# gabry1998/Self-Supervised-Anomaly-Detection

Measured on AMD Instinct MI355X. Metric: train images/sec + anomaly-maps/sec, ResNet-18 256x256 bs256, higher is better.
Workload: dtype f32; 1 GPU; ResNet-18 256x256 bs256 self-sup train + anomaly map, 1xMI355X, synthetic images (BASELINE configs[1]); images_per_gpu=256, global_batch=256, patches_per_image=841, bank_rows=588, parallelism=dp1 (256 images), train_step_launch=hipGraph segments, train_graph_segments=1

## Files before the change

include/ssad.h:

```cpp
#ifndef SSAD_H
#define SSAD_H
#include <stddef.h>
#include <stdint.h>

#ifdef __cplusplus
extern "C" {
#endif

#define SSAD_VERSION 100

int ssad_version(void);
const char* ssad_last_error(void);

int ssad_repack_oihw_to_ohwi(const float* w_oihw, float* w_ohwi, int O, int I, int KH, int KW, void* stream);
int ssad_repack_ohwi_to_oihw(const float* w_ohwi, float* w_oihw, int O, int I, int KH, int KW, void* stream);
int ssad_pack_stem_weight(const float* w_oihw, float* wk, void* stream);
int ssad_pack_stem_weight_ohwi(const float* w_ohwi, float* wk, void* stream);

int ssad_stem_fwd(const float* img, int B, int H, int W, int patch_dim, int patch_stride, int Hv, int Wv,
                  const float* wk, const float* scale, const float* shift, int relu, int hwnc, float* out, void* stream);
int ssad_stem_stats_rows(void);
int ssad_stem_fwd_stats(const float* img, int B, int H, int W, int Hv, int Wv, const float* wk, float* out, float eps,
                        float momentum, float* mean, float* invstd, float* running_mean, float* running_var, double* workspace,
                        void* stream);
// ... 3 lines not shown
                             const float* shift, int hwnc, float* out, void* stream);
int ssad_stem_patch_pool_fwd_ring(const float* img, int B, int H, int W, int patch_stride, const float* wf, const float* scale,
                                  const float* shift, int hwnc, int skip_lo, int skip_hi, float* out, void* stream);
int ssad_stem_patch_border_fwd(const float* img, int B, int H, int W, int patch_stride, const float* wf, const float* scale,
                               const float* shift, float* out, void* stream);

int ssad_maxpool3x3s2_fwd(const float* in, float* out, int64_t N, int H, int W, int C, int hwnc, void* stream);

int ssad_conv_igemm_fwd(const float* in, const float* w_ohwi, float* out, const float* scale, const float* shift,
                        const float* residual, int relu, int64_t N, int H, int W, int Cin, int Cout, int KH, int KW,
                        int stride, int pad, void* stream);

int ssad_conv_igemm_fwd_hwnc(const float* in, const float* w_ohwi, float* out, const float* scale, const float* shift,
                             const float* residual, int relu, int64_t N, int H, int W, int Cin, int Cout, int KH, int KW,
                             int stride, int pad, void* stream);

int ssad_conv_igemm_fwd_hwnc_ring(const float* in, const float* w_ohwi, float* out, const float* scale, const float* shift,
                                  const float* residual, int relu, int64_t N, int H, int W, int Cin, int Cout, int KH, int KW,
                                  int stride, int pad, int skip_lo, int skip_hi, void* stream);
int ssad_patch_gather_hwnc(const float* dense, float* out, int64_t B, int prow, int pcol, int shift, int Hd, int Wd, int C,
                           int H, int W, int lo, int hi, void* stream);
int ssad_patch_gather_hwnc_band(const float* dense, float* out, int64_t B, int prow, int pcol, int shift, int Hd, int Wd, int C,
                                int H, int W, int lo, int hi, int ilo, int ihi, void* stream);

int ssad_conv_igemm_tile(int64_t N, int H, int W, int Cin, int Cout, int KH, int KW, int stride, int pad, int mode);
int ssad_conv_igemm_tile_id(int64_t N, int H, int W, int Cin, int Cout, int KH, int KW, int stride, int pad, int mode);

int ssad_gap_fwd(const float* in, float* out, int64_t N, int HW, int C, int out_stride, int out_offset, int hwnc,
                 void* stream);

int ssad_l2_normalize_rows(const float* x, float* out, int64_t N, int D, void* stream);
int ssad_cosine_knn_mean(const float* sim, float* out, int64_t Nq, int Nb, int k, void* stream);

int ssad_blur_relu_bilinear(const float* maps, float* out, int n, int h, int w, int ksize, int target, void* stream);

int ssad_gradcam_map(const float* act, const float* alpha, float* out, int64_t B, int HW, int C, int alpha_stride,
                     void* stream);

int64_t ssad_auroc_workspace(int64_t n);
int ssad_auroc(const float* scores, const uint8_t* labels, int64_t n, void* workspace, int64_t workspace_bytes, double* out,
               void* stream);

int ssad_flip_transpose_weight(const float* w_ohwi, float* out, int O, int I, int KH, int KW, void* stream);
int ssad_flip_transpose_batch(const float* src, float* dst, const int64_t* desc, int n, void* stream);
int ssad_conv_igemm_dgrad(const float* dy, const float* w_flipT, float* dx, const float* residual, int64_t N, int Hy, int Wy,
                          int Cout, int Hx, int Wx, int Cin, int KH, int KW, int stride, int pad, void* stream);
// ... 310 lines not shown
```

self-supervised-anomaly-detection_amd/csrc/conv_igemm.hip:

```cpp
#include "common.h"
#include <stdlib.h>
#include <type_traits>

#ifndef IGEMM_ABL
#define IGEMM_ABL 0
#endif
#ifndef IGEMM_VAR
#define IGEMM_VAR 4
#endif
#ifndef IGEMM_EPI
#define IGEMM_EPI 1
#endif


#ifndef IGEMM_BUFLD
#define IGEMM_BUFLD 1
#endif

#ifndef IGEMM_TRACE
#define IGEMM_TRACE 0
#endif
#if IGEMM_TRACE
__device__ unsigned long long* g_ig_trace;
#define IG_STAMP(i) do { if (threadIdx.x == 0 && g_ig_trace) g_ig_trace[((size_t)blockIdx.y * gridDim.x + blockIdx.x) * 8 + (i)] = __builtin_readcyclecounter(); } while (0)
// ... 4 lines not shown
namespace {

constexpr int KALIGN = 32;

__device__ __attribute__((aligned(16))) float g_zero_page[8] = {0, 0, 0, 0, 0, 0, 0, 0};

struct ConvParams {
    const float* in;
    const float* wt;
    float* out;
    const float* scale;
    const float* shift;
    const float* residual;
    const uint8_t* res_mask;
    int64_t M;
    int64_t N;
    int H, W, Cin, Ho, Wo, Cout, KH, KW, stride, pad, relu;
    int K;
    int hwnc;
    int cls_start[5];
    int cls_id[4];
    double* stats;
    int skip_lo, skip_hi;
    int pos_lpt;
    int pos_sg;
    int pos_chunk;
    unsigned char pos_tab[64];
};

template <int BM, int BN, int TM, int TN, int BK, int TS, bool POS, bool DB = true, int BF = 0, bool IO = false>
__global__ __launch_bounds__((BM / (32 * TM)) * (BN / (32 * TN)) * 64, (TM * TN > 8 || (TM * TN == 8 && BK >= 32)) ? 1 : 2)
void conv_igemm_f32_kernel(ConvParams p) {
    static_assert(!IO || BF == 2, "half tensors go with fp16 operands");
    using io_t = std::conditional_t<IO, hf, float>;
    constexpr int PE = IO ? 8 : 4;
    constexpr int NT = (BM / (32 * TM)) * (BN / (32 * TN)) * 64;
    constexpr int LDK = BF == 6 ? 3 * BK + 8 : (BF == 3 ? 2 * BK + 8 : (BF ? BK + 8 : BK + 4));
    constexpr int ESZ = BF ? 2 : 4;
    constexpr int CPR = BK / PE;
    constexpr int RPP = NT / CPR;
    constexpr int WN = BN / (32 * TN);
    constexpr int AR = BM / RPP;
    constexpr int BR = BN / RPP;
    static_assert(AR >= 1 && BR >= 1, "tile too small for the staging pattern");
    constexpr int STAGE = (BM + BN) * LDK * ESZ / 4;
    constexpr int LDC = BN + 4;
// ... 29 lines not shown
            const unsigned pi = r / (unsigned)p.pos_chunk, g = r - pi * (unsigned)p.pos_chunk;
            const unsigned sg = (blk * (unsigned)p.pos_chunk + g) * 8u + x;
            if (sg >= (unsigned)p.pos_sg) return;
            pos = p.pos_tab[pi];
            m0 = (int64_t)sg * BM;
        } else if (p.pos_lpt) {
            const unsigned per_chunk = (unsigned)p.pos_chunk * (unsigned)HoWo;
            const unsigned chunk = blockIdx.x / per_chunk, in_chunk = blockIdx.x - chunk * per_chunk;
            const unsigned first = chunk * (unsigned)p.pos_chunk;
            const unsigned here = min((unsigned)p.pos_chunk, (unsigned)p.pos_sg - first);
            const unsigned pi = in_chunk / here;
            if (pi >= (unsigned)HoWo) return;
            pos = p.pos_tab[pi];
            m0 = (int64_t)(first + in_chunk - pi * here) * BM;
        } else {
        const int stream = blockIdx.x & 31;
        const int64_t j = blockIdx.x >> 5;
        const int64_t q = j / HoWo;
        pos = (int)(j - q * HoWo);
        m0 = (q * 32 + stream) * BM;
        }
        if (m0 >= p.N) return;
        const int oy = pos / p.Wo, ox = pos - oy * p.Wo;
        if (oy >= p.skip_lo && oy <= p.skip_hi && ox >= p.skip_lo && ox <= p.skip_hi) return;
        tapmask = 0;
        for (int ky = 0, t = 0; ky < p.KH; ++ky)
            for (int kx = 0; kx < p.KW; ++kx, ++t) {
                const int y = oy * p.stride - p.pad + ky, x = ox * p.stride - p.pad + kx;
                if ((unsigned)y < (unsigned)p.H && (unsigned)x < (unsigned)p.W) tapmask |= 1u << t;
            }
    } else {
        m0 = (int64_t)blockIdx.x * BM;
    }
    int cpy = 0, cpx = 0, Hc = 1, Wc = 1;
    int64_t Mc = 0;
    if (TS > 1) {
        int c = 0;
        while (c < 3 && (int)blockIdx.x >= p.cls_start[c + 1]) ++c;
        cpy = p.cls_id[c] >> 1;
        cpx = p.cls_id[c] & 1;
        Hc = (p.Ho - cpy + 1) / 2;
        Wc = (p.Wo - cpx + 1) / 2;
        Mc = p.N * Hc * Wc;
        m0 = (int64_t)((int)blockIdx.x - p.cls_start[c]) * BM;
        tapmask = 0;
        for (int ky = 0, t = 0; ky < p.KH; ++ky)
            for (int kx = 0; kx < p.KW; ++kx, ++t)
// ... 803 lines not shown
        return launch<128, 128, 2, 2, 32, TS, POS, false, 6>(p, st);
    }
    if (p.Cout <= 64) return launch<256, 64, 2, 2, 16, TS, POS, true, 6>(p, st);
    return launch<128, 128, 2, 2, 16, TS, POS, true, 6>(p, st);
}

template <int TS, bool POS>
int dispatch_x3(const ConvParams& p, hipStream_t st) {
    static const int v = getenv("SSAD_X3_VARIANT") ? atoi(getenv("SSAD_X3_VARIANT")) : 1;
    if (v == 1) {
        if (p.Cout <= 64) return launch<256, 64, 2, 2, 32, TS, POS, false, 3>(p, st);
        return launch<128, 128, 2, 2, 32, TS, POS, false, 3>(p, st);
    }
    if (p.Cout <= 64) return launch<256, 64, 2, 2, 16, TS, POS, true, 3>(p, st);
    return launch<128, 128, 2, 2, 32, TS, POS, true, 3>(p, st);
}

enum IgemmTile { T_256x64_K16 = 0, T_256x64_SB, T_128x64, T_256x128, T_256x128_W4, T_128x256, T_64x64, T_128x128, T_256x256, T_128x64_SB, T_128x64_K16, T_128x128_K16, T_128x256_K16 };

template <bool POS>
IgemmTile pick_tile(const ConvParams& p) {
    static const int variant = getenv("SSAD_CONV64_VARIANT") ? atoi(getenv("SSAD_CONV64_VARIANT")) : 1;
    static const int ring = getenv("SSAD_CONV_RING_VARIANT") ? atoi(getenv("SSAD_CONV_RING_VARIANT")) : 0;
    if (p.Cout <= 64 && POS && p.skip_lo <= p.skip_hi && !getenv("SSAD_CONV64_VARIANT"))
        return ring == 1 ? T_128x64_SB : ring == 3 ? T_128x64 : T_128x64_K16;
    if (p.Cout <= 64) return variant == 2 ? T_256x64_SB : variant == 1 ? T_256x64_K16 : T_128x64;
    static const int big = getenv("SSAD_CONV128_VARIANT") ? atoi(getenv("SSAD_CONV128_VARIANT")) : 0;
    if (big == 7) return T_128x128_K16;
    if (big == 1) return T_256x128;
    if (big == 2) return T_256x128_W4;
    if (big == 6 && POS && p.Cout % 256 == 0 && cdiv64(p.N, 256) * p.Ho * p.Wo * (p.Cout / 256) >= 256) return T_256x256;
    static const int wide_min = getenv("SSAD_CONV_WIDE_GRID") ? atoi(getenv("SSAD_CONV_WIDE_GRID")) : 256;
    if (big != 5 && p.Cout % 256 == 0 && wide_min > 0) {
        const int64_t rows = POS ? cdiv64(p.N, 128) * p.Ho * p.Wo : cdiv64(p.M, 128);
        static const int wide_k16 = getenv("SSAD_CONV256_K16") ? atoi(getenv("SSAD_CONV256_K16")) : 2;
        if (rows * (p.Cout / 256) >= wide_min) return (wide_k16 == 2 || (POS && wide_k16)) ? T_128x256_K16 : T_128x256;
    }
    static const int small_min = getenv("SSAD_CONV_SMALL_GRID") ? atoi(getenv("SSAD_CONV_SMALL_GRID")) : 500;
    static const int tiny_min = getenv("SSAD_CONV_TINY_GRID") ? atoi(getenv("SSAD_CONV_TINY_GRID")) : 520;
    if (!POS) {
        const int64_t g128 = cdiv64(p.M, 128) * ((p.Cout + 127) / 128);
        if (cdiv64(p.M, 128) * ((p.Cout + 63) / 64) < tiny_min && p.M > 128) return T_64x64;
        if (g128 < small_min) return T_128x64;
    }
    static const int k16 = getenv("SSAD_CONV128_K16") ? atoi(getenv("SSAD_CONV128_K16")) : 1;
    if (POS && k16) return T_128x128_K16;
    return T_128x128;
// ... 10 lines not shown
        case T_128x128_K16: return launch<128, 128, 2, 2, 16, TS, POS>(p, st);
        case T_128x256_K16: return launch<128, 256, 2, 4, 16, TS, POS>(p, st);
        case T_256x128: return launch<256, 128, 2, 2, 32, TS, POS>(p, st);
        case T_256x128_W4: return launch<256, 128, 4, 2, 32, TS, POS>(p, st);
        case T_128x256: return launch<128, 256, 2, 4, 32, TS, POS>(p, st);
        case T_64x64: return launch<64, 64, 1, 1, 32, TS, POS>(p, st);
        case T_256x256:
            if constexpr (POS && TS == 1) return launch<256, 256, 4, 4, 32, TS, POS>(p, st);
            else return launch<128, 128, 2, 2, 32, TS, POS>(p, st);
        default: return launch<128, 128, 2, 2, 32, TS, POS>(p, st);
    }
}

enum IgemmEntry { E_FWD = 0, E_HWNC = 1, E_RING = 2, E_STATS = 3, E_DGRAD = 4 };

static bool posmajor_rows(IgemmEntry e, const ConvParams& p) {
    if (e == E_HWNC || e == E_RING) return true;
    return e == E_FWD && p.pad > 0 && p.N >= 128 && p.Ho * p.Wo <= 4;
}

static ConvParams dgrad_params(int64_t N, int Hy, int Wy, int Cout, int Hx, int Wx, int Cin, int KH, int KW, int pad) {
    ConvParams p;
    p.pos_lpt = 0; p.pos_sg = 0; p.pos_chunk = 1;
    p.skip_lo = 1; p.skip_hi = 0;
    p.in = nullptr; p.wt = nullptr; p.out = nullptr; p.scale = nullptr; p.shift = nullptr; p.residual = nullptr; p.res_mask = nullptr;
    p.H = Hy; p.W = Wy; p.Cin = Cout; p.Cout = Cin; p.KH = KH; p.KW = KW; p.relu = 0;
    p.stride = 1; p.pad = KH - 1 - pad; p.N = N; p.hwnc = 0;
    p.Ho = Hx; p.Wo = Wx; p.stats = nullptr;
    p.M = N * Hx * Wx;
    p.K = KH * KW * Cout;
    return p;
}

static bool tile_span_ok(const ConvParams& p, bool posmajor, int elt_bytes, int ts = 1) {
    const int64_t image = (int64_t)p.H * p.W * p.Cin * elt_bytes;
    if (posmajor) return p.hwnc || 256 * image < ((int64_t)1 << 31);
    const int64_t rows_per_image = ts > 1 ? (int64_t)(p.Ho / 2) * (p.Wo / 2) : (int64_t)p.Ho * p.Wo;
    return (256 / (rows_per_image > 0 ? rows_per_image : 1) + 2) * image < ((int64_t)1 << 31);
}

int conv_fwd_impl(const float* in, const float* w_ohwi, float* out, const float* scale, const float* shift,
                  const float* residual, int relu, int64_t N, int H, int W, int Cin, int Cout, int KH, int KW, int stride,
                  int pad, int hwnc, void* stream, int bf16 = 0, double* stats = nullptr, int* stat_rows = nullptr, int io16 = 0,
                  int skip_lo = 1, int skip_hi = 0) {
    SSAD_CHECK_ARG(in && w_ohwi && out, "null pointer");
    SSAD_CHECK_ARG(!io16 || (bf16 == 2 && !hwnc && Cout % 4 == 0), "half tensors: fp16 operands, NHWC, Cout % 4 == 0");
    SSAD_CHECK_ARG(N > 0 && H > 0 && W > 0 && Cin > 0 && Cout > 0, "empty shape");
    if ((bf16 == 0 || bf16 == 1 || bf16 == 2) && !io16 && !hwnc && KH == 1 && KW == 1 && H == 1 && W == 1 && stride == 1 && pad == 0 &&
        ssad_linear_small_ok(in, w_ohwi, N, Cin))
        return ssad_linear_small_launch(in, w_ohwi, out, scale, shift, residual, relu, (int)N, Cin, Cout, stats, stat_rows, stream, bf16);
    SSAD_CHECK_ARG(Cin % KALIGN == 0, "Cin must be a multiple of 32");
    SSAD_CHECK_ARG(KH > 0 && KW > 0 && stride > 0 && pad >= 0 && KH * KW <= 32, "bad filter geometry (<= 32 taps)");
    ConvParams p;
    p.pos_lpt = 0; p.pos_sg = 0; p.pos_chunk = 1;
    p.skip_lo = skip_lo; p.skip_hi = skip_hi;
    SSAD_CHECK_ARG(skip_lo > skip_hi || hwnc, "a skipped rectangle of output positions: position-major tensors only");
    p.in = in; p.wt = w_ohwi; p.out = out; p.scale = scale; p.shift = shift; p.residual = residual; p.res_mask = nullptr;
    p.H = H; p.W = W; p.Cin = Cin; p.Cout = Cout; p.KH = KH; p.KW = KW; p.stride = stride; p.pad = pad; p.relu = relu;
    p.Ho = (H + 2 * pad - KH) / stride + 1;
    p.Wo = (W + 2 * pad - KW) / stride + 1;
    SSAD_CHECK_ARG(p.Ho > 0 && p.Wo > 0, "empty output");
    p.M = N * p.Ho * p.Wo;
    p.N = N;
    p.K = KH * KW * Cin;
    p.hwnc = hwnc;
    p.stats = stats;
    const bool posmajor = posmajor_rows(hwnc ? (skip_lo <= skip_hi ? E_RING : E_HWNC) : stats ? E_STATS : E_FWD, p);
    SSAD_CHECK_ARG(cdiv64(p.M, 128) + 32 * p.Ho * p.Wo < (int64_t)2147483647, "M too large for one launch");
    SSAD_CHECK_ARG(tile_span_ok(p, posmajor, io16 ? 2 : 4), "input images too large: the rows of a tile must span less than 2 GB");
    hipStream_t st = (hipStream_t)stream;
    int rows;
    SSAD_CHECK_ARG(bf16 == 0 || bf16 == 1 || bf16 == 2 || bf16 == 3 || bf16 == 6,
                   "operand mode: 0 (fp32), 1 (bf16), 2 (fp16), 3 (bf16x3), 6 (bf16x6)");
    if (bf16 == 6) {
        rows = posmajor ? dispatch_x6<1, true>(p, st) : dispatch_x6<1, false>(p, st);
    } else if (bf16 == 3) {
        rows = posmajor ? dispatch_x3<1, true>(p, st) : dispatch_x3<1, false>(p, st);
    } else if (bf16) {
        SSAD_CHECK_ARG(!hwnc, "16-bit operands: NHWC only");
        rows = io16 ? dispatch_bf16<1, 2, true>(p, st) : bf16 == 2 ? dispatch_bf16<1, 2>(p, st) : dispatch_bf16<1, 1>(p, st);
    } else if (posmajor) rows = dispatch<1, true>(p, st);
    else rows = dispatch<1, false>(p, st);
    if (stat_rows) *stat_rows = rows;
    SSAD_CHECK_LAUNCH();
    return 0;
}

}

extern "C" int ssad_conv_igemm_fwd_bf16(const float* in, const float* w_ohwi, float* out, const float* scale,
// ... 39 lines not shown
    int rc = conv_fwd_impl(in, w_ohwi, out, nullptr, nullptr, nullptr, 0, N, H, W, Cin, Cout, KH, KW, stride, pad, 0, stream,
                           bf16, workspace, &rows);
    if (rc) return rc;
    const int Ho = (H + 2 * pad - KH) / stride + 1, Wo = (W + 2 * pad - KW) / stride + 1;
    return ssad_bn_finalize_partials(workspace, rows, N * Ho * Wo, Cout, eps, momentum, mean, invstd, running_mean,
                                     running_var, stream);
}

extern "C" int ssad_conv_igemm_fwd_hwnc(const float* in, const float* w_ohwi, float* out, const float* scale,
                                        const float* shift, const float* residual, int relu, int64_t N, int H, int W,
                                        int Cin, int Cout, int KH, int KW, int stride, int pad, void* stream) {
    return conv_fwd_impl(in, w_ohwi, out, scale, shift, residual, relu, N, H, W, Cin, Cout, KH, KW, stride, pad, 1, stream);
}

extern "C" int ssad_conv_igemm_fwd_hwnc_ring(const float* in, const float* w_ohwi, float* out, const float* scale,
                                             const float* shift, const float* residual, int relu, int64_t N, int H, int W,
                                             int Cin, int Cout, int KH, int KW, int stride, int pad, int skip_lo, int skip_hi,
                                             void* stream) {
    SSAD_CHECK_ARG(skip_lo >= 0 && skip_hi < H && skip_hi < W, "skipped square outside the map");
    return conv_fwd_impl(in, w_ohwi, out, scale, shift, residual, relu, N, H, W, Cin, Cout, KH, KW, stride, pad, 1, stream, 0, nullptr,
                         nullptr, 0, skip_lo, skip_hi);
}

extern "C" int ssad_conv_igemm_tile_id(int64_t N, int H, int W, int Cin, int Cout, int KH, int KW, int stride, int pad, int mode) {
    const int Ho = (H + 2 * pad - KH) / stride + 1, Wo = (W + 2 * pad - KW) / stride + 1;
    ConvParams p;
    if (mode == E_DGRAD) {
        p = dgrad_params(N, Ho, Wo, Cout, H, W, Cin, KH, KW, pad);
    } else {
        p.N = N; p.H = H; p.W = W; p.Cin = Cin; p.Cout = Cout; p.KH = KH; p.KW = KW; p.stride = stride; p.pad = pad;
        p.skip_lo = mode == E_RING ? 0 : 1; p.skip_hi = 0;
        p.Ho = Ho; p.Wo = Wo;
        p.M = N * p.Ho * p.Wo;
    }
    if (posmajor_rows((IgemmEntry)mode, p)) return 100 + (int)pick_tile<true>(p);
    const IgemmTile t = pick_tile<false>(p);
    return t == T_256x256 ? T_128x128 : (int)t;
}

extern "C" int ssad_conv_igemm_tile(int64_t N, int H, int W, int Cin, int Cout, int KH, int KW, int stride, int pad, int mode) {
    static const int dims[13][3] = {{256, 64, 16}, {256, 64, 32}, {128, 64, 32}, {256, 128, 32}, {256, 128, 32}, {128, 256, 32},
                                    {64, 64, 32}, {128, 128, 32}, {256, 256, 32}, {128, 64, 32}, {128, 64, 16}, {128, 128, 16}, {128, 256, 16}};
    const int id = ssad_conv_igemm_tile_id(N, H, W, Cin, Cout, KH, KW, stride, pad, mode), t = id % 100;
    const int code = dims[t][0] * 100000 + dims[t][1] * 100 + dims[t][2];
    return id >= 100 ? -code : code;
}

static int dgrad_impl(const float* dy, const float* w_flipT, float* dx, const float* residual, int64_t N,
                                     int Hy, int Wy, int Cout, int Hx, int Wx, int Cin, int KH, int KW, int stride,
                                     int pad, void* stream, int bf16, const uint8_t* res_mask = nullptr, int io16 = 0) {
    SSAD_CHECK_ARG(dy && w_flipT && dx, "null pointer");
    SSAD_CHECK_ARG(!io16 || (bf16 == 2 && !res_mask && Cin % 4 == 0), "half tensors: fp16 operands, no residual mask, Cin % 4 == 0");
    SSAD_CHECK_ARG(N > 0 && Hy > 0 && Wy > 0 && Hx > 0 && Wx > 0 && Cin > 0 && Cout > 0, "empty shape");
    if ((bf16 == 0 || bf16 == 1 || bf16 == 2) && !io16 && !res_mask && KH == 1 && KW == 1 && Hy == 1 && Wy == 1 && Hx == 1 && Wx == 1 &&
// ... 95 lines not shown
```

self-supervised-anomaly-detection_amd/csrc/misc.hip:

```cpp
#include "common.h"
#include <stdarg.h>

static thread_local char g_err[512] = "";

void ssad_set_error(const char* fmt, ...) {
    va_list ap;
    va_start(ap, fmt);
    vsnprintf(g_err, sizeof(g_err), fmt, ap);
    va_end(ap);
}

extern "C" const char* ssad_last_error(void) { return g_err; }
extern "C" int ssad_version(void) { return 100; }

namespace {

__global__ void repack_kernel(const float* __restrict__ src, float* __restrict__ dst, int O, int I, int KH, int KW,
                              int to_ohwi) {
    int64_t idx = (int64_t)blockIdx.x * blockDim.x + threadIdx.x;
    int64_t total = (int64_t)O * I * KH * KW;
    if (idx >= total) return;
    int ci = (int)(idx % I);
    int64_t t = idx / I;
    int kx = (int)(t % KW); t /= KW;
// ... 297 lines not shown
}

extern "C" int ssad_patch_gather_hwnc_band(const float* dense, float* out, int64_t B, int prow, int pcol, int shift, int Hd, int Wd, int C,
                                           int H, int W, int lo, int hi, int ilo, int ihi, void* stream) {
    SSAD_CHECK_ARG(dense && out && B > 0 && prow > 0 && pcol > 0 && shift > 0 && C > 0 && C % 4 == 0, "bad argument");
    SSAD_CHECK_ARG(lo >= 0 && hi >= lo && hi < H && hi < W, "the copied square must lie inside the map");
    SSAD_CHECK_ARG(ilo > ihi || (ilo > lo && ihi < hi), "the inner square must lie strictly inside the copied one");
    SSAD_CHECK_ARG(shift * (prow - 1) + hi < Hd && shift * (pcol - 1) + hi < Wd, "the dense map does not cover the last patch");
    const int64_t N = B * prow * pcol;
    const int side = hi - lo + 1;
    const int iside = ilo > ihi ? 0 : ihi - ilo + 1;
    SSAD_CHECK_ARG(cdiv64(N * (C / 4), 256) < (int64_t)2147483647 && side * side <= 65535, "too large for one launch");
    hipLaunchKernelGGL(patch_gather_hwnc_kernel, dim3((unsigned)cdiv64(N * (C / 4), 256), side * side - iside * iside), dim3(256), 0,
                       (hipStream_t)stream, (const f32x4*)dense, (f32x4*)out, N, prow, pcol, shift, Hd, Wd, C / 4, W, lo, side, ilo, iside);
    SSAD_CHECK_LAUNCH();
    return 0;
}

extern "C" int ssad_patch_gather_hwnc(const float* dense, float* out, int64_t B, int prow, int pcol, int shift, int Hd, int Wd, int C,
                                      int H, int W, int lo, int hi, void* stream) {
    return ssad_patch_gather_hwnc_band(dense, out, B, prow, pcol, shift, Hd, Wd, C, H, W, lo, hi, 1, 0, stream);
}

extern "C" int ssad_gradcam_map(const float* act, const float* alpha, float* out, int64_t B, int HW, int C, int alpha_stride,
                                void* stream) {
    SSAD_CHECK_ARG(act && alpha && out && B > 0 && HW > 0 && C > 0 && alpha_stride >= C, "bad argument");
    const int64_t rows = B * HW;
    hipLaunchKernelGGL(gradcam_map_kernel, dim3((unsigned)cdiv64(rows, 4)), dim3(256), 0, (hipStream_t)stream, act, alpha, out,
                       rows, HW, C, alpha_stride);
    SSAD_CHECK_LAUNCH();
    return 0;
}

extern "C" int ssad_l2_normalize_rows(const float* x, float* out, int64_t N, int D, void* stream) {
    SSAD_CHECK_ARG(x && out && N > 0 && D > 0, "bad argument");
    hipLaunchKernelGGL(l2norm_rows_kernel, dim3((unsigned)cdiv64(N, 4)), dim3(256), 0, (hipStream_t)stream, x, out, N, D);
    SSAD_CHECK_LAUNCH();
    return 0;
}

extern "C" int ssad_cosine_knn_mean(const float* sim, float* out, int64_t Nq, int Nb, int k, void* stream) {
    SSAD_CHECK_ARG(sim && out && Nq > 0 && Nb > 0, "bad argument");
    SSAD_CHECK_ARG(k >= 1 && k <= 3 && k <= Nb, "k must be 1..3 and <= bank rows");
    hipLaunchKernelGGL(knn_mean_kernel, dim3((unsigned)cdiv64(Nq, 4)), dim3(256), 0, (hipStream_t)stream, sim, out, Nq, Nb, k);
    SSAD_CHECK_LAUNCH();
    return 0;
// ... 25 lines not shown
```

self-supervised-anomaly-detection_amd/self_supervised/_hip.py:

```python
import ctypes
import os

import torch

_HERE = os.path.dirname(os.path.abspath(__file__))
LIB_PATH = os.path.join(os.path.dirname(_HERE), "lib", "libssad_hip.so")

_c_fp = ctypes.c_void_p
_c_i = ctypes.c_int
_c_l = ctypes.c_int64
_c_f = ctypes.c_float

SIGNATURES = {
    "ssad_repack_oihw_to_ohwi": [_c_fp, _c_fp, _c_i, _c_i, _c_i, _c_i, _c_fp],
    "ssad_repack_ohwi_to_oihw": [_c_fp, _c_fp, _c_i, _c_i, _c_i, _c_i, _c_fp],
    "ssad_pack_stem_weight": [_c_fp, _c_fp, _c_fp],
    "ssad_pack_stem_weight_ohwi": [_c_fp, _c_fp, _c_fp],
    "ssad_pack_stem_weight16_ohwi": [_c_fp, _c_fp, _c_i, _c_fp],
    "ssad_stem_fwd": [_c_fp, _c_i, _c_i, _c_i, _c_i, _c_i, _c_i, _c_i, _c_fp, _c_fp, _c_fp, _c_i, _c_i, _c_fp, _c_fp],
    "ssad_stem_stats_rows": [],
    "ssad_stem_fwd_stats": [_c_fp, _c_i, _c_i, _c_i, _c_i, _c_i, _c_fp, _c_fp, _c_f, _c_f, _c_fp, _c_fp, _c_fp, _c_fp, _c_fp, _c_fp],
    "ssad_pack_stem_weight_folded": [_c_fp, _c_fp, _c_fp],
    "ssad_stem_patch_pool_fwd": [_c_fp, _c_i, _c_i, _c_i, _c_i, _c_fp, _c_fp, _c_fp, _c_i, _c_fp, _c_fp],
    "ssad_stem_patch_pool_fwd_ring": [_c_fp, _c_i, _c_i, _c_i, _c_i, _c_fp, _c_fp, _c_fp, _c_i, _c_i, _c_i, _c_fp, _c_fp],
    "ssad_stem_patch_border_fwd": [_c_fp, _c_i, _c_i, _c_i, _c_i, _c_fp, _c_fp, _c_fp, _c_fp, _c_fp],
    "ssad_maxpool3x3s2_fwd": [_c_fp, _c_fp, _c_l, _c_i, _c_i, _c_i, _c_i, _c_fp],
    "ssad_conv_igemm_fwd": [_c_fp, _c_fp, _c_fp, _c_fp, _c_fp, _c_fp, _c_i, _c_l, _c_i, _c_i, _c_i, _c_i, _c_i, _c_i,
                            _c_i, _c_i, _c_fp],
    "ssad_conv_igemm_fwd_hwnc": [_c_fp, _c_fp, _c_fp, _c_fp, _c_fp, _c_fp, _c_i, _c_l, _c_i, _c_i, _c_i, _c_i, _c_i, _c_i,
                                 _c_i, _c_i, _c_fp],
    "ssad_conv_igemm_fwd_hwnc_ring": [_c_fp, _c_fp, _c_fp, _c_fp, _c_fp, _c_fp, _c_i, _c_l, _c_i, _c_i, _c_i, _c_i, _c_i, _c_i,
                                      _c_i, _c_i, _c_i, _c_i, _c_fp],
    "ssad_patch_gather_hwnc": [_c_fp, _c_fp, _c_l, _c_i, _c_i, _c_i, _c_i, _c_i, _c_i, _c_i, _c_i, _c_i, _c_i, _c_fp],
    "ssad_patch_gather_hwnc_band": [_c_fp, _c_fp, _c_l, _c_i, _c_i, _c_i, _c_i, _c_i, _c_i, _c_i, _c_i, _c_i, _c_i, _c_i, _c_i, _c_fp],
    "ssad_conv_igemm_tile": [_c_l, _c_i, _c_i, _c_i, _c_i, _c_i, _c_i, _c_i, _c_i, _c_i],
    "ssad_conv_igemm_tile_id": [_c_l, _c_i, _c_i, _c_i, _c_i, _c_i, _c_i, _c_i, _c_i, _c_i],
    "ssad_gap_fwd": [_c_fp, _c_fp, _c_l, _c_i, _c_i, _c_i, _c_i, _c_i, _c_fp],
    "ssad_l2_normalize_rows": [_c_fp, _c_fp, _c_l, _c_i, _c_fp],
    "ssad_cosine_knn_mean": [_c_fp, _c_fp, _c_l, _c_i, _c_i, _c_fp],
    "ssad_cosine_knn_fused": [_c_fp, _c_fp, _c_fp, _c_l, _c_i, _c_i, _c_i, _c_fp],
    "ssad_cosine_knn_split": [_c_fp, _c_fp, _c_fp, _c_fp, _c_l, _c_i, _c_i, _c_i, _c_i, _c_fp],
    "ssad_cosine_knn_index": [_c_fp, _c_fp, _c_fp, _c_fp, _c_l, _c_i, _c_i, _c_i, _c_fp],
    "ssad_cosine_knn_index_split": [_c_fp, _c_fp, _c_fp, _c_fp, _c_fp, _c_l, _c_i, _c_i, _c_i, _c_i, _c_fp],
    "ssad_rows_smallest_index": [_c_fp, _c_l, _c_i, _c_i, _c_i, _c_i, _c_fp, _c_fp, _c_fp, _c_fp],
    "ssad_rows_argmax": [_c_fp, _c_l, _c_i, _c_fp, _c_fp, _c_fp],
    "ssad_knn_reweight": [_c_fp, _c_fp, _c_fp, _c_fp, _c_fp, _c_fp, _c_l, _c_i, _c_i, _c_i, _c_fp],
    "ssad_row_sqnorms": [_c_fp, _c_fp, _c_l, _c_i, _c_fp],
    "ssad_l2_knn_fused": [_c_fp, _c_fp, _c_fp, _c_fp, _c_l, _c_i, _c_i, _c_i, _c_fp],
    "ssad_l2_knn_split": [_c_fp, _c_fp, _c_fp, _c_fp, _c_fp, _c_l, _c_i, _c_i, _c_i, _c_i, _c_fp],
    "ssad_l2_knn_index": [_c_fp, _c_fp, _c_fp, _c_fp, _c_fp, _c_l, _c_i, _c_i, _c_i, _c_fp],
    "ssad_l2_knn_index_split": [_c_fp, _c_fp, _c_fp, _c_fp, _c_fp, _c_fp, _c_l, _c_i, _c_i, _c_i, _c_i, _c_fp],
    "ssad_l2_from_dots": [_c_fp, _c_fp, _c_fp, _c_fp, _c_l, _c_i, _c_fp],
    "ssad_knn_reweight_l2": [_c_fp, _c_fp, _c_fp, _c_fp, _c_fp, _c_fp, _c_l, _c_i, _c_i, _c_i, _c_fp],
    "ssad_local_patch_features": [_c_fp, _c_fp, _c_fp, _c_l, _c_i, _c_i, _c_i, _c_i, _c_i, _c_i, _c_i, _c_fp],
    "ssad_coreset_greedy": [_c_fp, _c_l, _c_i, _c_i, _c_l, _c_i, _c_fp, _c_fp, _c_fp, _c_fp, _c_fp, _c_fp],
# ... 215 lines not shown
```

self-supervised-anomaly-detection_amd/self_supervised/engine.py:

```python
import torch
from torch import nn

import os as _os

from . import ops

BLOCKS = [("layer1", 64, 64, 1), ("layer2", 64, 128, 2), ("layer3", 128, 256, 2), ("layer4", 256, 512, 2)]


def math_mode():
    m = _os.environ.get("SSAD_MATH", "f32").lower()
    return 6 if m in ("bf16x6", "x6") else 3 if m in ("bf16x3", "x3") else 0


class _Block(nn.Module):

    def __init__(self, cin, cout, stride):
        super().__init__()
        self.conv1 = nn.Conv2d(cin, cout, 3, stride, 1, bias=False)
        self.bn1 = nn.BatchNorm2d(cout)
        self.conv2 = nn.Conv2d(cout, cout, 3, 1, 1, bias=False)
        self.bn2 = nn.BatchNorm2d(cout)
        self.downsample = None
        if stride != 1 or cin != cout:
# ... 126 lines not shown
        if last_of_stage and maps is not None and name in maps:
            maps[name] = a
    return pooled


def _trunk_eval_dedup(plan, x, patch_stride, layer_outputs, pooled, conv):
    b, _, h, w = x.shape
    prow, pcol = (h - 32) // patch_stride + 1, (w - 32) // patch_stride + 1
    shift = patch_stride // 2
    band = _os.environ.get("SSAD_GATHER_BAND", "1") != "0"
    dn = ops.stem_fwd(x, plan.stem_w, plan.stem_s, plan.stem_t, True, resize_to=(2 * h, 2 * w))
    dn = ops.maxpool3x3s2_fwd(dn)
    if band and _os.environ.get("SSAD_STEM_BORDER", "1") != "0":
        a = ops.stem_patch_border_fwd(x, plan.stem_wf, plan.stem_s, plan.stem_t, patch_stride)
        ops.patch_gather_hwnc(dn, a, prow, pcol, shift, 2, 14, 4, 12)
    else:
        a = ops.stem_patch_pool_fwd(x, plan.stem_wf, plan.stem_s, plan.stem_t, patch_stride, True, (4, 12) if band else None)
    offs, off = {}, 0
    for k in ("layer1", "layer2", "layer3"):
        if k in layer_outputs:
            offs[k] = off
            off += {"layer1": 64, "layer2": 128, "layer3": 256}[k]
    offs["layer4"] = off
    for i, (name, d) in enumerate(plan.blocks):
        s = d["stride"]
        if name == "layer1":
            lo, hi = 3 + 2 * i, 13 - 2 * i
            dt = ops.conv3x3_c64_eval(dn, d["w1"], d["s1"], d["t1"], None, True)
            dn2 = ops.conv3x3_c64_eval(dt, d["w2"], d["s2"], d["t2"], dn, True)
            t = ops.conv_fwd_hwnc_ring(a, d["w1"], d["s1"], d["t1"], None, True, lo, hi)
            ops.patch_gather_hwnc(dt, t, prow, pcol, shift, lo, hi, *((lo + 2, hi - 2) if band else (1, 0)))
            a2 = ops.conv_fwd_hwnc_ring(t, d["w2"], d["s2"], d["t2"], a, True, lo + 1, hi - 1)
            ops.patch_gather_hwnc(dn2, a2, prow, pcol, shift, lo + 1, hi - 1, *((lo + 3, hi - 3) if band and i == 0 else (1, 0)))
            a, dn = a2, dn2
        else:
            idt = a
            if "wd" in d:
                idt = conv(a, d["wd"], d["sd"], d["td"], None, False, s, 0)
            t = conv(a, d["w1"], d["s1"], d["t1"], None, True, s, 1)
            a = conv(t, d["w2"], d["s2"], d["t2"], idt, True, 1, 1)
        if i % 2 == 1 and name in offs:
            ops.gap_fwd(a, pooled, offs[name], True)
    return pooled


def head_eval(plan, pooled):
    f = pooled
    x3 = math_mode()
    for w, s, t, relu in plan.head:
        f = ops.linear_fwd(f, w, s, t, relu, x3)
    logits = ops.linear_fwd(f, plan.cls_w, None, plan.cls_b, False, x3)
    return logits, f
```

self-supervised-anomaly-detection_amd/self_supervised/ops.py:

```python
import os

import torch

from . import _hip


PROFILE = None


def _new(shape, like):
    return torch.empty(shape, device=like.device, dtype=torch.float32)


def _newh(shape, like):
    return torch.empty(shape, device=like.device, dtype=torch.float16)


def _is_h(t):
    return t is not None and t.dtype == torch.float16


def _p(t, allow_none=False):
    return _hip.ptr(t, allow_none, torch.float16 if _is_h(t) else torch.float32)

# ... 250 lines not shown
         lambda: _hip.lib().ssad_conv_igemm_fwd_hwnc(_hip.ptr(x), _hip.ptr(w_ohwi), _hip.ptr(out), _hip.ptr(scale, True),
                                                     _hip.ptr(shift, True), _hip.ptr(residual, True), int(relu), n, h, w,
                                                     cin, cout, kh, kw, stride, pad, _hip.stream()),
         exec_flops=2.0 * n * cout * cin * _inbounds_taps(h, w, kh, kw, stride, pad) if PROFILE is not None else None,
         tile=lambda: igemm_tile_name(n, h, w, cin, cout, kh, kw, stride, pad, IGEMM_HWNC))
    return out


def conv_fwd_hwnc_ring(x, w_ohwi, scale, shift, residual, relu, skip_lo, skip_hi):
    h, w, n, cin = x.shape
    cout, kh, kw, cin2 = w_ohwi.shape
    assert cin == cin2 and (kh, kw) == (3, 3) and 0 <= skip_lo <= skip_hi < min(h, w)
    out = _new((h, w, n, cout), x)
    side = skip_hi - skip_lo + 1
    ring = h * w - side * side
    taps = _inbounds_taps(h, w, 3, 3, 1, 1) - 9 * side * side if PROFILE is not None else 0
    _run("conv_igemm_pos_f32", 2.0 * n * ring * cout * 9 * cin, 4.0 * (x.numel() + n * ring * cout * (2 if residual is not None else 1) + w_ohwi.numel()),
         lambda: _hip.lib().ssad_conv_igemm_fwd_hwnc_ring(_hip.ptr(x), _hip.ptr(w_ohwi), _hip.ptr(out), _hip.ptr(scale, True),
                                                          _hip.ptr(shift, True), _hip.ptr(residual, True), int(relu), n, h, w,
                                                          cin, cout, 3, 3, 1, 1, skip_lo, skip_hi, _hip.stream()),
         exec_flops=2.0 * n * cout * cin * taps if PROFILE is not None else None,
         tile=lambda: igemm_tile_name(n, h, w, cin, cout, 3, 3, 1, 1, IGEMM_RING))
    return out


def patch_gather_hwnc(dense, out, prow, pcol, shift, lo, hi, ilo=1, ihi=0):
    b, hd, wd, c = dense.shape
    h, w, n, c2 = out.shape
    assert c == c2 and n == b * prow * pcol
    side, iside = hi - lo + 1, max(ihi - ilo + 1, 0)
    _run("patch_gather", 0.0, 8.0 * n * (side * side - iside * iside) * c,
         lambda: _hip.lib().ssad_patch_gather_hwnc_band(_hip.ptr(dense), _hip.ptr(out), b, prow, pcol, shift, hd, wd, c, h, w, lo, hi,
                                                        ilo, ihi, _hip.stream()))
    return out


def conv_fwd(x, w_ohwi, scale=None, shift=None, residual=None, relu=False, stride=1, pad=0, bf16=False):
    n, h, w, cin = x.shape
    cout, kh, kw, cin2 = w_ohwi.shape
    assert cin == cin2
    ho, wo = (h + 2 * pad - kh) // stride + 1, (w + 2 * pad - kw) // stride + 1
    out = _new((n, ho, wo, cout), x)
    nb = 4.0 * (x.numel() + out.numel() * (2 if residual is not None else 1) + w_ohwi.numel())
    if bf16 in (3, 6):
        _run("conv_igemm_x6" if bf16 == 6 else "conv_igemm_x3", 2.0 * out.numel() * kh * kw * cin, nb,
             lambda: _split_fwd(bf16)(_hip.ptr(x), _hip.ptr(w_ohwi), _hip.ptr(out), _hip.ptr(scale, True),
# ... 1111 lines not shown
```

Measured before the change: 8205 images/sec.

## Share overlapping patch-edge conv outputs across neighboring patches in layer1 eval

Adds a position-masked ring conv together with gather and replicate kernels so that layer1 edge positions shared between horizontally or vertically overlapping patches are computed once per patch row or column and then copied to the neighbours. This removes redundant conv work on the halo ring during patch-level anomaly-map evaluation. In exchange it launches more, smaller kernels and adds copy traffic, and correctness depends on the edge activations of overlapping patches being exactly identical.

After: 8210 images/sec, median of 2. Within noise of the previous version (+0.1%).

```diff
diff --git a/include/ssad.h b/include/ssad.h
--- a/include/ssad.h
+++ b/include/ssad.h
@@ -49,6 +49,14 @@
                            int H, int W, int lo, int hi, void* stream);
 int ssad_patch_gather_hwnc_band(const float* dense, float* out, int64_t B, int prow, int pcol, int shift, int Hd, int Wd, int C,
                                 int H, int W, int lo, int hi, int ilo, int ihi, void* stream);
+
+int ssad_conv_igemm_fwd_hwnc_masked(const float* in, const float* w_ohwi, float* out, const float* scale, const float* shift,
+                                    const float* residual, int relu, int64_t N, int H, int W, int Cin, int Cout, int KH, int KW,
+                                    int stride, int pad, uint64_t m0, uint64_t m1, uint64_t m2, uint64_t m3, void* stream);
+int ssad_patch_rows_gather_hwnc(const float* in, float* out, int64_t B, int prow, int pcol, int by_col, int C, int H, int W,
+                                uint64_t m0, uint64_t m1, uint64_t m2, uint64_t m3, void* stream);
+int ssad_patch_edge_replicate_hwnc(float* t, const float* crow, const float* ccol, int64_t B, int prow, int pcol, int shift, int C,
+                                   int H, int W, int lo, int hi, void* stream);
 
 int ssad_conv_igemm_tile(int64_t N, int H, int W, int Cin, int Cout, int KH, int KW, int stride, int pad, int mode);
 int ssad_conv_igemm_tile_id(int64_t N, int H, int W, int Cin, int Cout, int KH, int KW, int stride, int pad, int mode);
diff --git a/self-supervised-anomaly-detection_amd/csrc/conv_igemm.hip b/self-supervised-anomaly-detection_amd/csrc/conv_igemm.hip
--- a/self-supervised-anomaly-detection_amd/csrc/conv_igemm.hip
+++ b/self-supervised-anomaly-detection_amd/csrc/conv_igemm.hip
@@ -50,6 +50,8 @@
     int cls_id[4];
     double* stats;
     int skip_lo, skip_hi;
+    int use_mask;
+    uint64_t pos_mask[4];
     int pos_lpt;
     int pos_sg;
     int pos_chunk;
@@ -125,7 +127,9 @@
         }
         if (m0 >= p.N) return;
         const int oy = pos / p.Wo, ox = pos - oy * p.Wo;
-        if (oy >= p.skip_lo && oy <= p.skip_hi && ox >= p.skip_lo && ox <= p.skip_hi) return;
+        if (p.use_mask) {
+            if (!((p.pos_mask[pos >> 6] >> (pos & 63)) & 1)) return;
+        } else if (oy >= p.skip_lo && oy <= p.skip_hi && ox >= p.skip_lo && ox <= p.skip_hi) return;
         tapmask = 0;
         for (int ky = 0, t = 0; ky < p.KH; ++ky)
             for (int kx = 0; kx < p.KW; ++kx, ++t) {
@@ -975,7 +979,7 @@
 IgemmTile pick_tile(const ConvParams& p) {
     static const int variant = getenv("SSAD_CONV64_VARIANT") ? atoi(getenv("SSAD_CONV64_VARIANT")) : 1;
     static const int ring = getenv("SSAD_CONV_RING_VARIANT") ? atoi(getenv("SSAD_CONV_RING_VARIANT")) : 0;
-    if (p.Cout <= 64 && POS && p.skip_lo <= p.skip_hi && !getenv("SSAD_CONV64_VARIANT"))
+    if (p.Cout <= 64 && POS && (p.skip_lo <= p.skip_hi || p.use_mask) && !getenv("SSAD_CONV64_VARIANT"))
         return ring == 1 ? T_128x64_SB : ring == 3 ? T_128x64 : T_128x64_K16;
     if (p.Cout <= 64) return variant == 2 ? T_256x64_SB : variant == 1 ? T_256x64_K16 : T_128x64;
     static const int big = getenv("SSAD_CONV128_VARIANT") ? atoi(getenv("SSAD_CONV128_VARIANT")) : 0;
@@ -1032,7 +1036,7 @@
 static ConvParams dgrad_params(int64_t N, int Hy, int Wy, int Cout, int Hx, int Wx, int Cin, int KH, int KW, int pad) {
     ConvParams p;
     p.pos_lpt = 0; p.pos_sg = 0; p.pos_chunk = 1;
-    p.skip_lo = 1; p.skip_hi = 0;
+    p.skip_lo = 1; p.skip_hi = 0; p.use_mask = 0;
     p.in = nullptr; p.wt = nullptr; p.out = nullptr; p.scale = nullptr; p.shift = nullptr; p.residual = nullptr; p.res_mask = nullptr;
     p.H = Hy; p.W = Wy; p.Cin = Cout; p.Cout = Cin; p.KH = KH; p.KW = KW; p.relu = 0;
     p.stride = 1; p.pad = KH - 1 - pad; p.N = N; p.hwnc = 0;
@@ -1052,7 +1056,7 @@
 int conv_fwd_impl(const float* in, const float* w_ohwi, float* out, const float* scale, const float* shift,
                   const float* residual, int relu, int64_t N, int H, int W, int Cin, int Cout, int KH, int KW, int stride,
                   int pad, int hwnc, void* stream, int bf16 = 0, double* stats = nullptr, int* stat_rows = nullptr, int io16 = 0,
-                  int skip_lo = 1, int skip_hi = 0) {
+                  int skip_lo = 1, int skip_hi = 0, const uint64_t* pos_mask = nullptr) {
     SSAD_CHECK_ARG(in && w_ohwi && out, "null pointer");
     SSAD_CHECK_ARG(!io16 || (bf16 == 2 && !hwnc && Cout % 4 == 0), "half tensors: fp16 operands, NHWC, Cout % 4 == 0");
     SSAD_CHECK_ARG(N > 0 && H > 0 && W > 0 && Cin > 0 && Cout > 0, "empty shape");
@@ -1065,6 +1069,9 @@
     p.pos_lpt = 0; p.pos_sg = 0; p.pos_chunk = 1;
     p.skip_lo = skip_lo; p.skip_hi = skip_hi;
     SSAD_CHECK_ARG(skip_lo > skip_hi || hwnc, "a skipped rectangle of output positions: position-major tensors only");
+    p.use_mask = pos_mask != nullptr;
+    for (int i = 0; i < 4; ++i) p.pos_mask[i] = pos_mask ? pos_mask[i] : 0;
+    SSAD_CHECK_ARG(!pos_mask || (hwnc && !bf16 && skip_lo > skip_hi), "a mask of output positions: exact fp32, position-major tensors only");
     p.in = in; p.wt = w_ohwi; p.out = out; p.scale = scale; p.shift = shift; p.residual = residual; p.res_mask = nullptr;
     p.H = H; p.W = W; p.Cin = Cin; p.Cout = Cout; p.KH = KH; p.KW = KW; p.stride = stride; p.pad = pad; p.relu = relu;
     p.Ho = (H + 2 * pad - KH) / stride + 1;
@@ -1075,7 +1082,8 @@
     p.K = KH * KW * Cin;
     p.hwnc = hwnc;
     p.stats = stats;
-    const bool posmajor = posmajor_rows(hwnc ? (skip_lo <= skip_hi ? E_RING : E_HWNC) : stats ? E_STATS : E_FWD, p);
+    SSAD_CHECK_ARG(!pos_mask || p.Ho * p.Wo <= 256, "a mask of output positions: maps of at most 256 positions");
+    const bool posmajor = posmajor_rows(hwnc ? (skip_lo <= skip_hi || pos_mask ? E_RING : E_HWNC) : stats ? E_STATS : E_FWD, p);
     SSAD_CHECK_ARG(cdiv64(p.M, 128) + 32 * p.Ho * p.Wo < (int64_t)2147483647, "M too large for one launch");
     SSAD_CHECK_ARG(tile_span_ok(p, posmajor, io16 ? 2 : 4), "input images too large: the rows of a tile must span less than 2 GB");
     hipStream_t st = (hipStream_t)stream;
@@ -1161,6 +1169,15 @@
                          nullptr, 0, skip_lo, skip_hi);
 }
 
+extern "C" int ssad_conv_igemm_fwd_hwnc_masked(const float* in, const float* w_ohwi, float* out, const float* scale,
+                                               const float* shift, const float* residual, int relu, int64_t N, int H, int W,
+                                               int Cin, int Cout, int KH, int KW, int stride, int pad, uint64_t m0, uint64_t m1,
+                                               uint64_t m2, uint64_t m3, void* stream) {
+    const uint64_t mask[4] = {m0, m1, m2, m3};
+    return conv_fwd_impl(in, w_ohwi, out, scale, shift, residual, relu, N, H, W, Cin, Cout, KH, KW, stride, pad, 1, stream, 0, nullptr,
+                         nullptr, 0, 1, 0, mask);
+}
+
 extern "C" int ssad_conv_igemm_tile_id(int64_t N, int H, int W, int Cin, int Cout, int KH, int KW, int stride, int pad, int mode) {
     const int Ho = (H + 2 * pad - KH) / stride + 1, Wo = (W + 2 * pad - KW) / stride + 1;
     ConvParams p;
@@ -1169,6 +1186,7 @@
     } else {
         p.N = N; p.H = H; p.W = W; p.Cin = Cin; p.Cout = Cout; p.KH = KH; p.KW = KW; p.stride = stride; p.pad = pad;
         p.skip_lo = mode == E_RING ? 0 : 1; p.skip_hi = 0;
+        p.use_mask = 0;
         p.Ho = Ho; p.Wo = Wo;
         p.M = N * p.Ho * p.Wo;
     }
diff --git a/self-supervised-anomaly-detection_amd/csrc/misc.hip b/self-supervised-anomaly-detection_amd/csrc/misc.hip
--- a/self-supervised-anomaly-detection_amd/csrc/misc.hip
+++ b/self-supervised-anomaly-detection_amd/csrc/misc.hip
@@ -343,6 +343,84 @@
     return ssad_patch_gather_hwnc_band(dense, out, B, prow, pcol, shift, Hd, Wd, C, H, W, lo, hi, 1, 0, stream);
 }
 
+namespace {
+struct PosMask { uint64_t w[4]; };
+__global__ __launch_bounds__(256) void patch_rows_gather_kernel(const f32x4* __restrict__ in, f32x4* __restrict__ out, int64_t N, int64_t R,
+                                                                int prow, int pcol, int by_col, int C4, PosMask mask) {
+    const int pos = (int)blockIdx.y;
+    if (!((mask.w[pos >> 6] >> (pos & 63)) & 1)) return;
+    const int64_t i = (int64_t)blockIdx.x * 256 + threadIdx.x;
+    if (i >= R * C4) return;
+    const int c4 = (int)(i % C4);
+    const int64_t r = i / C4;
+    const int64_t n = by_col ? (r / pcol) * prow * pcol + r % pcol : r * pcol;
+    out[((int64_t)pos * R + r) * C4 + c4] = in[((int64_t)pos * N + n) * C4 + c4];
+}
+
+__global__ __launch_bounds__(256) void patch_edge_replicate_kernel(f32x4* t, const f32x4* __restrict__ crow,
+                                                                   const f32x4* __restrict__ ccol, int64_t N, int prow, int pcol, int shift,
+                                                                   int C4, int H, int W, int lo, int hi) {
+    const int64_t i = (int64_t)blockIdx.x * 256 + threadIdx.x;
+    if (i >= N * C4) return;
+    const int c4 = (int)(i % C4);
+    const int64_t n = i / C4;
+    const int pp = prow * pcol;
+    const int64_t b = n / pp;
+    const int rem = (int)(n - b * pp);
+    const int pr = rem / pcol, pc = rem - pr * pcol;
+    const int side = hi - lo + 1, span = side - shift;
+    int k = (int)blockIdx.y;
+    const int nrow = (H - side) * span;
+    int u, v;
+    const f32x4* src;
+    if (k < nrow) {
+        const int q = k / span;
+        u = q < lo ? q : q + side;
+        v = lo + k % span;
+        const int kmax = (hi - v) / shift;
+        if (pc >= kmax) src = t + (((int64_t)u * W + v + kmax * shift) * N + n - kmax) * C4 + c4;
+        else src = crow + (((int64_t)u * W + v + pc * shift) * (N / pcol) + b * prow + pr) * C4 + c4;
+    } else {
+        k -= nrow;
+        const int q = k / span;
+        v = q < lo ? q : q + side;
+        u = lo + k % span;
+        const int kmax = (hi - u) / shift;
+        if (pr >= kmax) src = t + (((int64_t)(u + kmax * shift) * W + v) * N + n - (int64_t)kmax * pcol) * C4 + c4;
+        else src = ccol + (((int64_t)(u + pr * shift) * W + v) * (N / prow) + b * pcol + pc) * C4 + c4;
+    }
+    t[(((int64_t)u * W + v) * N + n) * C4 + c4] = *src;
+}
+}
+
+extern "C" int ssad_patch_rows_gather_hwnc(const float* in, float* out, int64_t B, int prow, int pcol, int by_col, int C, int H, int W,
+                                           uint64_t m0, uint64_t m1, uint64_t m2, uint64_t m3, void* stream) {
+    SSAD_CHECK_ARG(in && out && B > 0 && prow > 0 && pcol > 0 && C > 0 && C % 4 == 0 && H > 0 && W > 0, "bad argument");
+    SSAD_CHECK_ARG(H * W <= 256, "a mask of positions: maps of at most 256 positions");
+    const int64_t N = B * prow * pcol, R = B * (by_col ? pcol : prow);
+    SSAD_CHECK_ARG(cdiv64(R * (C / 4), 256) < (int64_t)2147483647, "too large for one launch");
+    PosMask mask = {{m0, m1, m2, m3}};
+    hipLaunchKernelGGL(patch_rows_gather_kernel, dim3((unsigned)cdiv64(R * (C / 4), 256), H * W), dim3(256), 0, (hipStream_t)stream,
+                       (const f32x4*)in, (f32x4*)out, N, R, prow, pcol, by_col, C / 4, mask);
+    SSAD_CHECK_LAUNCH();
+    return 0;
+}
+
+extern "C" int ssad_patch_edge_replicate_hwnc(float* t, const float* crow, const float* ccol, int64_t B, int prow, int pcol, int shift, int C,
+                                              int H, int W, int lo, int hi, void* stream) {
+    SSAD_CHECK_ARG(t && crow && ccol && B > 0 && prow > 0 && pcol > 0 && shift > 0 && C > 0 && C % 4 == 0, "bad argument");
+    SSAD_CHECK_ARG(lo >= 0 && hi >= lo && hi < H && hi < W, "the interior square must lie inside the map");
+    const int side = hi - lo + 1, span = side - shift;
+    SSAD_CHECK_ARG(span > 0, "interior not wider than the shift: no edge position is shared");
+    const int64_t N = B * prow * pcol;
+    const int ny = (H - side + W - side) * span;
+    SSAD_CHECK_ARG(ny > 0 && ny <= 65535 && cdiv64(N * (C / 4), 256) < (int64_t)2147483647, "nothing to copy, or too large for one launch");
+    hipLaunchKernelGGL(patch_edge_replicate_kernel, dim3((unsigned)cdiv64(N * (C / 4), 256), ny), dim3(256), 0, (hipStream_t)stream,
+                       (f32x4*)t, (const f32x4*)crow, (const f32x4*)ccol, N, prow, pcol, shift, C / 4, H, W, lo, hi);
+    SSAD_CHECK_LAUNCH();
+    return 0;
+}
+
 extern "C" int ssad_gradcam_map(const float* act, const float* alpha, float* out, int64_t B, int HW, int C, int alpha_stride,
                                 void* stream) {
     SSAD_CHECK_ARG(act && alpha && out && B > 0 && HW > 0 && C > 0 && alpha_stride >= C, "bad argument");
diff --git a/self-supervised-anomaly-detection_amd/self_supervised/_hip.py b/self-supervised-anomaly-detection_amd/self_supervised/_hip.py
--- a/self-supervised-anomaly-detection_amd/self_supervised/_hip.py
+++ b/self-supervised-anomaly-detection_amd/self_supervised/_hip.py
@@ -10,6 +10,7 @@
 _c_i = ctypes.c_int
 _c_l = ctypes.c_int64
 _c_f = ctypes.c_float
+_c_u64 = ctypes.c_uint64
 
 SIGNATURES = {
     "ssad_repack_oihw_to_ohwi": [_c_fp, _c_fp, _c_i, _c_i, _c_i, _c_i, _c_fp],
@@ -31,6 +32,10 @@
                                  _c_i, _c_i, _c_fp],
     "ssad_conv_igemm_fwd_hwnc_ring": [_c_fp, _c_fp, _c_fp, _c_fp, _c_fp, _c_fp, _c_i, _c_l, _c_i, _c_i, _c_i, _c_i, _c_i, _c_i,
                                       _c_i, _c_i, _c_i, _c_i, _c_fp],
+    "ssad_conv_igemm_fwd_hwnc_masked": [_c_fp, _c_fp, _c_fp, _c_fp, _c_fp, _c_fp, _c_i, _c_l, _c_i, _c_i, _c_i, _c_i, _c_i, _c_i,
+                                        _c_i, _c_i, _c_u64, _c_u64, _c_u64, _c_u64, _c_fp],
+    "ssad_patch_rows_gather_hwnc": [_c_fp, _c_fp, _c_l, _c_i, _c_i, _c_i, _c_i, _c_i, _c_i, _c_u64, _c_u64, _c_u64, _c_u64, _c_fp],
+    "ssad_patch_edge_replicate_hwnc": [_c_fp, _c_fp, _c_fp, _c_l, _c_i, _c_i, _c_i, _c_i, _c_i, _c_i, _c_i, _c_i, _c_fp],
     "ssad_patch_gather_hwnc": [_c_fp, _c_fp, _c_l, _c_i, _c_i, _c_i, _c_i, _c_i, _c_i, _c_i, _c_i, _c_i, _c_i, _c_fp],
     "ssad_patch_gather_hwnc_band": [_c_fp, _c_fp, _c_l, _c_i, _c_i, _c_i, _c_i, _c_i, _c_i, _c_i, _c_i, _c_i, _c_i, _c_i, _c_i, _c_fp],
     "ssad_conv_igemm_tile": [_c_l, _c_i, _c_i, _c_i, _c_i, _c_i, _c_i, _c_i, _c_i, _c_i],
diff --git a/self-supervised-anomaly-detection_amd/self_supervised/engine.py b/self-supervised-anomaly-detection_amd/self_supervised/engine.py
--- a/self-supervised-anomaly-detection_amd/self_supervised/engine.py
+++ b/self-supervised-anomaly-detection_amd/self_supervised/engine.py
@@ -172,16 +172,25 @@
             offs[k] = off
             off += {"layer1": 64, "layer2": 128, "layer3": 256}[k]
     offs["layer4"] = off
+    es = _EdgeShare(b, prow, pcol, shift, a) if _os.environ.get("SSAD_EDGE_SHARE", "1") != "0" else None
     for i, (name, d) in enumerate(plan.blocks):
         s = d["stride"]
         if name == "layer1":
             lo, hi = 3 + 2 * i, 13 - 2 * i
             dt = ops.conv3x3_c64_eval(dn, d["w1"], d["s1"], d["t1"], None, True)
             dn2 = ops.conv3x3_c64_eval(dt, d["w2"], d["s2"], d["t2"], dn, True)
-            t = ops.conv_fwd_hwnc_ring(a, d["w1"], d["s1"], d["t1"], None, True, lo, hi)
-            ops.patch_gather_hwnc(dt, t, prow, pcol, shift, lo, hi, *((lo + 2, hi - 2) if band else (1, 0)))
-            a2 = ops.conv_fwd_hwnc_ring(t, d["w2"], d["s2"], d["t2"], a, True, lo + 1, hi - 1)
-            ops.patch_gather_hwnc(dn2, a2, prow, pcol, shift, lo + 1, hi - 1, *((lo + 3, hi - 3) if band and i == 0 else (1, 0)))
+            inner1 = (lo + 2, hi - 2) if band else (1, 0)
+            inner2 = (lo + 3, hi - 3) if band and i == 0 else (1, 0)
+            if es is not None and es.shares(2 * i, lo, hi):
+                t = es.conv(a, d["w1"], d["s1"], d["t1"], False, dt, lo, hi, inner1)
+            else:
+                t = ops.conv_fwd_hwnc_ring(a, d["w1"], d["s1"], d["t1"], None, True, lo, hi)
+                ops.patch_gather_hwnc(dt, t, prow, pcol, shift, lo, hi, *inner1)
+            if es is not None and es.shares(2 * i + 1, lo + 1, hi - 1):
+                a2 = es.conv(t, d["w2"], d["s2"], d["t2"], True, dn2, lo + 1, hi - 1, inner2)
+            else:
+                a2 = ops.conv_fwd_hwnc_ring(t, d["w2"], d["s2"], d["t2"], a, True, lo + 1, hi - 1)
+                ops.patch_gather_hwnc(dn2, a2, prow, pcol, shift, lo + 1, hi - 1, *inner2)
             a, dn = a2, dn2
         else:
             idt = a
@@ -194,6 +203,41 @@
     return pooled
 
 
+class _EdgeShare:
+
+    def __init__(self, b, prow, pcol, shift, a):
+        self.b, self.prow, self.pcol, self.shift = b, prow, pcol, shift
+        self.convs = int(_os.environ.get("SSAD_EDGE_SHARE_CONVS", "4"))
+        self.row = self.col = self.row_in = self.col_in = None
+        if self.shares(0, 3, 13):
+            outer, inner = [q for q in range(16) if q < 4 or q > 12], range(2, 14 - shift + 1)
+            self.row = ops.patch_rows_gather_hwnc(a, b, prow, pcol, False, ops.position_mask(16, 16, [(u, v) for u in outer for v in inner]))
+            self.col = ops.patch_rows_gather_hwnc(a, b, prow, pcol, True, ops.position_mask(16, 16, [(u, v) for u in inner for v in outer]))
+
+    def shares(self, j, lo, hi):
+        return j < self.convs and hi - lo + 1 > self.shift and (j == 0 or self.row is not None)
+
+    def conv(self, x, w, s, t, residual, dense, lo, hi, inner):
+        b, prow, pcol, shift = self.b, self.prow, self.pcol, self.shift
+        outer = [q for q in range(16) if q < lo or q > hi]
+        fresh, shared = range(hi - shift + 1, hi + 1), range(lo, hi - shift + 1)
+        m_big = ops.position_mask(16, 16, [(u, v) for u in outer for v in outer] + [(u, v) for u in outer for v in fresh]
+                                  + [(u, v) for u in fresh for v in outer])
+        m_row = ops.position_mask(16, 16, [(u, v) for u in outer for v in shared])
+        m_col = ops.position_mask(16, 16, [(u, v) for u in shared for v in outer])
+        res = self.x_in if residual else (None, None, None)
+        y = ops.conv_fwd_hwnc_masked(x, w, s, t, res[0], True, m_big)
+        yr = ops.conv_fwd_hwnc_masked(self.row, w, s, t, res[1], True, m_row)
+        yc = ops.conv_fwd_hwnc_masked(self.col, w, s, t, res[2], True, m_col)
+        ops.patch_gather_hwnc(dense, y, prow, pcol, shift, lo, hi, *inner)
+        ops.patch_gather_hwnc(dense, yr, prow, 1, shift, lo, hi, *inner)
+        ops.patch_gather_hwnc(dense, yc, 1, pcol, shift, lo, hi, *inner)
+        ops.patch_edge_replicate_hwnc(y, yr, yc, b, prow, pcol, shift, lo, hi)
+        self.x_in = (x, self.row, self.col)
+        self.row, self.col = yr, yc
+        return y
+
+
 def head_eval(plan, pooled):
     f = pooled
     x3 = math_mode()
diff --git a/self-supervised-anomaly-detection_amd/self_supervised/ops.py b/self-supervised-anomaly-detection_amd/self_supervised/ops.py
--- a/self-supervised-anomaly-detection_amd/self_supervised/ops.py
+++ b/self-supervised-anomaly-detection_amd/self_supervised/ops.py
@@ -296,6 +296,61 @@
          exec_flops=2.0 * n * cout * cin * taps if PROFILE is not None else None,
          tile=lambda: igemm_tile_name(n, h, w, cin, cout, 3, 3, 1, 1, IGEMM_RING))
     return out
+
+
+def position_mask(h, w, positions):
+    m = 0
+    for u, v in positions:
+        assert 0 <= u < h and 0 <= v < w
+        m |= 1 << (u * w + v)
+    return m
+
+
+def _mask_words(mask):
+    assert 0 <= mask < 1 << 256
+    return [(mask >> (64 * i)) & 0xFFFFFFFFFFFFFFFF for i in range(4)]
+
+
+def conv_fwd_hwnc_masked(x, w_ohwi, scale, shift, residual, relu, mask):
+    h, w, n, cin = x.shape
+    cout, kh, kw, cin2 = w_ohwi.shape
+    assert cin == cin2 and (kh, kw) == (3, 3) and h * w <= 256
+    out = _new((h, w, n, cout), x)
+    npos = bin(mask).count("1")
+    taps = 0
+    if PROFILE is not None:
+        for pos in range(h * w):
+            if (mask >> pos) & 1:
+                u, v = divmod(pos, w)
+                taps += (3 - (u == 0) - (u == h - 1)) * (3 - (v == 0) - (v == w - 1))
+    _run("conv_igemm_pos_f32", 2.0 * n * npos * cout * 9 * cin, 4.0 * (x.numel() + n * npos * cout * (2 if residual is not None else 1) + w_ohwi.numel()),
+         lambda: _hip.lib().ssad_conv_igemm_fwd_hwnc_masked(_hip.ptr(x), _hip.ptr(w_ohwi), _hip.ptr(out), _hip.ptr(scale, True),
+                                                            _hip.ptr(shift, True), _hip.ptr(residual, True), int(relu), n, h, w,
+                                                            cin, cout, 3, 3, 1, 1, *_mask_words(mask), _hip.stream()),
+         exec_flops=2.0 * n * cout * cin * taps if PROFILE is not None else None,
+         tile=lambda: igemm_tile_name(n, h, w, cin, cout, 3, 3, 1, 1, IGEMM_RING))
+    return out
+
+
+def patch_rows_gather_hwnc(x, b, prow, pcol, by_col, mask):
+    h, w, n, c = x.shape
+    assert n == b * prow * pcol
+    r = b * (pcol if by_col else prow)
+    out = _new((h, w, r, c), x)
+    _run("patch_edge_copy", 0.0, 8.0 * r * bin(mask).count("1") * c,
+         lambda: _hip.lib().ssad_patch_rows_gather_hwnc(_hip.ptr(x), _hip.ptr(out), b, prow, pcol, int(by_col), c, h, w,
+                                                        *_mask_words(mask), _hip.stream()))
+    return out
+
+
+def patch_edge_replicate_hwnc(t, crow, ccol, b, prow, pcol, shift, lo, hi):
+    h, w, n, c = t.shape
+    assert n == b * prow * pcol and tuple(crow.shape) == (h, w, b * prow, c) and tuple(ccol.shape) == (h, w, b * pcol, c)
+    span = hi - lo + 1 - shift
+    _run("patch_edge_copy", 0.0, 8.0 * n * (h + w - 2 * (hi - lo + 1)) * span * c,
+         lambda: _hip.lib().ssad_patch_edge_replicate_hwnc(_hip.ptr(t), _hip.ptr(crow), _hip.ptr(ccol), b, prow, pcol, shift, c, h, w,
+                                                           lo, hi, _hip.stream()))
+    return t
 
 
 def patch_gather_hwnc(dense, out, prow, pcol, shift, lo, hi, ilo=1, ihi=0):
```
